# jdidion/atropos

Measured on AMD Instinct MI355X. Metric: reads/s (whole node) 150 bp SE adapter-align, higher is better.
Workload: dtype int32

## Files before the change

### atropos_amd/csrc/filter_core.hpp

```cpp
#ifndef ATR_FILTER_CORE_HPP
#define ATR_FILTER_CORE_HPP

#include "locate_core.hpp"

namespace atr {

constexpr int FILTER_MAX_M = 64;
constexpr int FILTER_CERT_T = 3;
constexpr int FILTER_CERT_TW = 6;
constexpr int FILTER_BINS = 256;

struct FilterParams {
    uint64_t peq[16];
    int rows;
    int and_mode;
    uint32_t tail;
    int32_t thr_row[FILTER_MAX_M + 1];
    uint32_t cert[FILTER_CERT_T + 1];
    uint64_t cert_sub;
    uint64_t rowsel[4];
    uint32_t tailx[3];
    uint64_t cert64[FILTER_CERT_TW + 1];
};

// ... 12 lines not shown
    const int R = m < rows ? m : rows;
    static thread_local uint8_t tab[FILTER_MAX_M + 1][FILTER_MAX_M + 1];
    uint32_t bad[FILTER_CERT_T + 1];
    for (int t = 0; t <= FILTER_CERT_T; ++t) bad[t] = 0u;
    for (int a = 1; a <= R; ++a) {
        const int xs = R - a;
        for (int y = 0; y <= R; ++y) tab[0][y] = 0;
        for (int x = 1; x <= xs; ++x) {
            tab[x][0] = 0;
            for (int y = 1; y <= R; ++y) {
                const uint8_t up = tab[x - 1][y], left = tab[x][y - 1];
                uint8_t v = up > left ? up : left;
                if (codes[a + x - 1] == codes[y - 1] && (uint8_t)(tab[x - 1][y - 1] + 1) > v) v = (uint8_t)(tab[x - 1][y - 1] + 1);
                tab[x][y] = v;
            }
        }
        for (int t = 1; t <= FILTER_CERT_T; ++t)
            for (int i = 1; i + t <= R && i < 32; ++i) {
                const int top = i + t, kk = thr_row[top];
                if (kk < t || a > top) continue;
                const int free_bases = t + kk;
                const int bound = (a < free_bases ? a : free_bases) + (int)tab[top - a][i];
                if (bound > i) bad[t] |= 1u << i;
            }
    }
    for (int t = 1; t <= FILTER_CERT_T; ++t)
        for (int i = 1; i + t <= R && i < 32; ++i)
            if (thr_row[i] >= 0 && thr_row[i + t] >= t && !((bad[t] >> i) & 1u)) cert[t] |= 1u << i;
}

inline void filter_overlap_certificates64(const uint8_t *codes, int m, int rows, const int32_t *thr_row, bool and_mode,
                                          uint64_t cert[FILTER_CERT_TW + 1]) {
    for (int t = 0; t <= FILTER_CERT_TW; ++t) cert[t] = 0ull;
    if (and_mode || rows <= 32 || rows > FILTER_MAX_M) return;
    const int R = m < rows ? m : rows;
    static thread_local uint8_t tab[FILTER_MAX_M + 1][FILTER_MAX_M + 1];
    uint64_t bad[FILTER_CERT_TW + 1];
    for (int t = 0; t <= FILTER_CERT_TW; ++t) bad[t] = 0ull;
    for (int a = 1; a <= R; ++a) {
        const int xs = R - a;
        for (int y = 0; y <= R; ++y) tab[0][y] = 0;
        for (int x = 1; x <= xs; ++x) {
            tab[x][0] = 0;
            for (int y = 1; y <= R; ++y) {
                const uint8_t up = tab[x - 1][y], left = tab[x][y - 1];
                uint8_t v = up > left ? up : left;
                if (codes[a + x - 1] == codes[y - 1] && (uint8_t)(tab[x - 1][y - 1] + 1) > v) v = (uint8_t)(tab[x - 1][y - 1] + 1);
                tab[x][y] = v;
            }
        }
        for (int t = 1; t <= FILTER_CERT_TW; ++t)
            for (int i = 1; i + t <= R && i < 64; ++i) {
                const int top = i + t, kk = thr_row[top];
                if (kk < t || a > top) continue;
                const int free_bases = t + kk;
                const int bound = (a < free_bases ? a : free_bases) + (int)tab[top - a][i];
                if (bound > i) bad[t] |= 1ull << i;
            }
    }
    for (int t = 1; t <= FILTER_CERT_TW; ++t)
        for (int i = 1; i + t <= R && i < 64; ++i)
            if (thr_row[i] >= 0 && thr_row[i + t] >= t && !((bad[t] >> i) & 1ull)) cert[t] |= 1ull << i;
}

inline uint64_t filter_substitution_certificate(const uint8_t *codes, int m, int k, bool and_mode) {
    if (and_mode || m < 8 || m > 64 || k < 1 || k > 4) return 0ull;
    for (int i = 0; i < m; ++i) if (codes[i] != 1 && codes[i] != 2 && codes[i] != 4 && codes[i] != 8) return 0ull;
    const int OLO = -3 * k, OHI = 2 * k, NO = OHI - OLO + 1;
    uint64_t cert = 0ull;
    for (int r = 1; r <= m; ++r) {
        const auto ok = [&](int i, int o) {
            const int q = i + o;
            if (q < 1 || q > m) return true;
            return q == r ? codes[i - 1] != codes[r - 1] : codes[i - 1] == codes[q - 1];
        };
        bool threat = false;
        {
            bool cur[24][5], nxt[24][5];
            for (int o = 0; o < NO; ++o) for (int b = 0; b <= k; ++b) cur[o][b] = (b == 0) && ok(1, OLO + o);
            for (int i = 2; i <= m; ++i) {
                for (int o = 0; o < NO; ++o) for (int b = 0; b <= k; ++b) nxt[o][b] = false;
                for (int o = 0; o < NO; ++o) for (int b = 0; b <= k; ++b) if (cur[o][b])
                    for (int step = 0; b + step <= k && o + step < NO; ++step) if (ok(i, OLO + o + step)) nxt[o + step][b + step] = true;
                for (int o = 0; o < NO; ++o) for (int b = 0; b <= k; ++b) cur[o][b] = nxt[o][b];
            }
            for (int o = 0; o < NO; ++o) for (int b = 0; b <= k; ++b) threat = threat || cur[o][b];
        }
        for (int o = -2 * k; o <= -1 && !threat; ++o) {
            int bad = 0;
            for (int i = 1; i <= m; ++i) bad += ok(i, o) ? 0 : 1;
            threat = bad <= 1;
        }
        for (int o = -2 * k; o <= 0 && !threat; ++o)
            for (int x = 1; x <= m && !threat; ++x) {
                bool all = true;
                for (int i = 1; i <= m && all; ++i) if (i != x) all = ok(i, i < x ? o : o - 1);
                threat = all;
            }
        if (!threat) cert |= 1ull << (r - 1);
    }
    return cert;
}

inline FilterParams filter_params(const uint64_t *peq64, const uint8_t *codes, int m, int flags, bool and_mode,
                                  const int16_t *thr, int min_overlap, bool planes_path = false) {
    FilterParams fp;
    fp.rows = m; fp.and_mode = and_mode ? 1 : 0; fp.tail = 0u;
    fp.tailx[0] = fp.tailx[1] = fp.tailx[2] = 0u;
    for (int i = 0; i <= FILTER_MAX_M; ++i)
        fp.thr_row[i] = (i >= 1 && i <= m && i >= min_overlap && ((flags & ATR_STOP_WITHIN_SEQ1) || i == m)) ? (int32_t)thr[i] : -1;
    for (int c = 0; c < 16; ++c) fp.peq[c] = peq64[c];
    (void)planes_path;
    if (filter_narrow_applies(m, flags)) {
        fp.rows = FILTER_NARROW_ROWS;
        for (int c = 0; c < 16; ++c) fp.peq[c] = (peq64[c] >> (64 - m)) & 0xFFFFFFFFull;
        for (int t = 0; t < m - FILTER_NARROW_ROWS; ++t) {
            const uint32_t nib = (uint32_t)(codes[FILTER_NARROW_ROWS + t] & 15u) << (4 * (t & 7));
            if (t < 8) fp.tail |= nib; else fp.tailx[(t >> 3) - 1] |= nib;
        }
    }
    filter_overlap_certificates(codes, m, fp.rows, fp.thr_row, and_mode, fp.cert);
    filter_overlap_certificates64(codes, m, planes_path ? fp.rows : 0, fp.thr_row, and_mode, fp.cert64);
    fp.cert_sub = 0ull;
    fp.rowsel[0] = fp.rowsel[1] = fp.rowsel[2] = fp.rowsel[3] = 0ull;
    if (m <= FILTER_MAX_M && (flags & ATR_STOP_WITHIN_SEQ2) && !(flags & ATR_START_WITHIN_SEQ1) && m >= min_overlap && thr[m] >= 1) {
        const int k = (int)thr[m];
        fp.cert_sub = filter_substitution_certificate(codes, m, k, and_mode);
        if (fp.cert_sub)
            for (int i = 0; i < m; ++i) fp.rowsel[codes[i] == 1 ? 0 : codes[i] == 2 ? 1 : codes[i] == 4 ? 2 : 3] |= 1ull << i;
    }
    return fp;
}

constexpr int BAND_W = 16;
#ifndef ATR_BAND_INTERSECT
#define ATR_BAND_INTERSECT 1
#endif
ATR_DEV uint32_t window_word(int j_lo, int j_hi, bool scan, int rows, bool band) {
    return 0x80000000u | (uint32_t)j_lo | ((uint32_t)j_hi << 10) | (scan ? (1u << 20) : 0u) | ((uint32_t)rows << 21) |
           (band ? (1u << 28) : 0u);
}
ATR_DEV bool window_band(uint32_t w) { return ((w >> 28) & 1u) != 0; }
ATR_DEV int window_rows(uint32_t w) { return (int)((w >> 21) & 0x7Fu); }
ATR_DEV int window_lo(uint32_t w) { return (int)(w & 0x3FFu); }
ATR_DEV int window_hi(uint32_t w) { return (int)((w >> 10) & 0x3FFu); }
ATR_DEV bool window_scan(uint32_t w) { return ((w >> 20) & 1u) != 0; }
ATR_DEV bool window_valid(uint32_t w) { return (w >> 31) != 0; }
ATR_DEV uint32_t last_band_word(int dlo, int top, int span, int width, bool rowm) {
    return window_word(dlo, span | (width << 6), true, top, true) | (rowm ? (1u << 29) : 0u);
}
ATR_DEV int last_band_span(uint32_t w) { return window_hi(w) & 63; }
ATR_DEV int last_band_width(uint32_t w) { return window_hi(w) >> 6; }
ATR_DEV bool last_band_rowm(uint32_t w) { return ((w >> 29) & 1u) != 0; }
constexpr int BAND_BINS = 96, ROWS_BIN0 = 192;
ATR_DEV int triangle_rows(int rows, int n, int j, int k) { return rows - (n - j) + k; }
ATR_DEV bool ragged_rows_bins(bool start_within_seq1) { return !start_within_seq1; }
constexpr int TAIL_COLUMNS = 64;

constexpr int LAST_BIN0 = 32;
ATR_DEV int window_bin(uint32_t w, int m, bool by_rows) {
    const int rows = window_rows(w), start = window_lo(w) >> 3;
    if (window_band(w)) {
        if (window_scan(w)) return LAST_BIN0 + 63 - atr_min(rows, 63);
        const int wide = atr_min(7, atr_max(0, (window_hi(w) - window_lo(w) - m) >> 1));
        return (7 - wide) * 4 + atr_min(3, start >> 4);
    }
    if (rows >= m || !by_rows) return 96 + start;
    return ROWS_BIN0 + atr_min(rows, 63);
}

#ifndef ATR_HOST_EMU
__device__ __forceinline__ void fetch_peq8(const uint2 *peq, uint32_t w, uint2 (&e)[8]) {
#pragma unroll
    for (int b = 0; b < 8; ++b) {
        uint32_t off;
        if (b == 0) off = (w << 3) & 0x78u;
        else asm("v_lshrrev_b32 %0, %1, %2\n\tv_and_b32 %0, 0x78, %0" : "=v"(off) : "n"(4 * b - 3), "v"(w));
        e[b] = *(const uint2 *)((const char *)peq + off);
    }
}
#endif

struct FilterState {
    uint32_t pvl, pvh, mvl, mvh;
    int score;
    uint32_t hits;
    uint32_t nz;
    int zfirst;
    int j_first, j_last;
};

ATR_DEV int filter_row_offset(int m, bool wide) { return (wide ? 64 : 32) - m; }
ATR_DEV int filter_row_offset(int m) { return filter_row_offset(m, m > 32); }

ATR_DEV void filter_init(FilterState &F, const Uniform &u, int mf, bool wide) {
    const int off = filter_row_offset(mf, wide);
    const uint32_t low = off >= 32 ? 0u : ~0u << (off & 31);
    if (wide) { F.pvl = u.sr ? 0u : low; F.pvh = u.sr ? 0u : (off > 32 ? ~0u << (off & 31) : ~0u); }
    else { F.pvl = u.sr ? 0u : low; F.pvh = 0u; }
    F.mvl = F.mvh = 0u;
    F.score = (u.sr ? 0 : mf) - (u.k + 1);
    F.hits = F.nz = 0u;
    F.zfirst = 0;
    F.j_first = F.j_last = 0;
}
ATR_DEV void filter_init(FilterState &F, const Uniform &u, int mf) { filter_init(F, u, mf, mf > 32); }

template <bool WIDE>
ATR_DEV void filter_shift_out2(uint32_t &phl, uint32_t &phh, uint32_t &mhl, uint32_t &mhh, int &score, uint32_t &hits,
                               uint32_t &nz, uint32_t kreg) {
#ifdef ATR_HOST_EMU
    hits = (hits << 1) | ((uint32_t)score >> 31);
    nz = (nz << 1) | (uint32_t)(((uint64_t)(uint32_t)score + (uint64_t)kreg) >> 32);
    const uint32_t pout = WIDE ? phh >> 31 : phl >> 31, mout = WIDE ? mhh >> 31 : mhl >> 31;
    if (WIDE) { phh = (phh << 1) | (phl >> 31); mhh = (mhh << 1) | (mhl >> 31); }
    phl <<= 1; mhl <<= 1;
    score += (int)pout - (int)mout;
#else
    uint64_t c0, c2, c3;
    uint32_t t1, t2;
    if (WIDE)
        asm("v_add_co_u32 %10, %8, %4, %4\n\t"
            "v_add_co_u32 %11, %9, %4, %12\n\t"
            "v_add_co_u32 %0, %7, %0, %0\n\t"
            "v_add_co_u32 %2, vcc, %2, %2\n\t"
            "v_addc_co_u32 %5, %8, %5, %5, %8\n\t"
            "v_addc_co_u32 %6, %9, %6, %6, %9\n\t"
            "v_addc_co_u32 %1, %7, %1, %1, %7\n\t"
            "v_addc_co_u32 %3, vcc, %3, %3, vcc\n\t"
            "s_nop 1\n\t"
            "v_addc_co_u32 %4, %7, 0, %4, %7\n\t"
            "v_subbrev_co_u32 %4, vcc, 0, %4, vcc"
            : "+v"(phl), "+v"(phh), "+v"(mhl), "+v"(mhh), "+v"(score), "+v"(hits), "+v"(nz), "=&s"(c0), "=&s"(c2), "=&s"(c3),
              "=&v"(t1), "=&v"(t2)
            : "v"(kreg) : "vcc");
    else
        asm("v_add_co_u32 %8, %6, %2, %2\n\t"
            "v_add_co_u32 %9, %7, %2, %10\n\t"
            "v_add_co_u32 %0, %5, %0, %0\n\t"
            "v_add_co_u32 %1, vcc, %1, %1\n\t"
            "v_addc_co_u32 %3, %6, %3, %3, %6\n\t"
            "v_addc_co_u32 %4, %7, %4, %4, %7\n\t"
            "v_addc_co_u32 %2, %5, 0, %2, %5\n\t"
            "v_subbrev_co_u32 %2, vcc, 0, %2, vcc"
            : "+v"(phl), "+v"(mhl), "+v"(score), "+v"(hits), "+v"(nz), "=&s"(c0), "=&s"(c2), "=&s"(c3), "=&v"(t1), "=&v"(t2)
            : "v"(kreg) : "vcc");
#endif
}

template <bool WIDE>
ATR_DEV void filter_step(FilterState &F, uint32_t eql, uint32_t eqh, uint32_t kreg) {
    const uint32_t xvl = eql | F.mvl;
    const uint32_t tl = eql & F.pvl;
    const uint32_t sl = tl + F.pvl;
    const uint32_t xhl = ((sl ^ F.pvl) | eql);
    uint32_t phl = F.mvl | ~(xhl | F.pvl);
    uint32_t mhl = F.pvl & xhl;
    uint32_t xvh = 0, phh = 0, mhh = 0;
    if (WIDE) {
        xvh = eqh | F.mvh;
        const uint32_t th = eqh & F.pvh;
        const uint32_t sh = th + F.pvh + (sl < tl ? 1u : 0u);
        const uint32_t xhh = ((sh ^ F.pvh) | eqh);
        phh = F.mvh | ~(xhh | F.pvh);
        mhh = F.pvh & xhh;
    }
    filter_shift_out2<WIDE>(phl, phh, mhl, mhh, F.score, F.hits, F.nz, kreg);
    F.pvl = mhl | ~(xvl | phl);
    F.mvl = phl & xvl;
    if (WIDE) {
        F.pvh = mhh | ~(xvh | phh);
        F.mvh = phh & xvh;
    }
}

ATR_DEV void filter_fold(FilterState &F, int j, int mf, uint32_t kreg) {
    F.hits = (F.hits << 1) | ((uint32_t)F.score >> 31);
    F.nz = (F.nz << 1) | ((uint32_t)F.score + kreg < kreg ? 1u : 0u);
    if (j < 32) { const uint32_t keep = j <= 0 ? 0u : (1u << j) - 1u; F.hits &= keep; F.nz &= keep; }
    if (F.hits != 0u) {
        const int hi = 31 - atr_clz(F.hits), lo = atr_ctz(F.hits);
        if (F.j_first == 0) F.j_first = j - hi;
        F.j_last = j - lo;
        if (F.zfirst == 0) {
            const int span = j - mf;
            const uint32_t ok = span >= 31 ? ~0u : span < 0 ? 0u : (2u << span) - 1u;
            const uint32_t z = F.hits & ~F.nz & ok;
            if (z != 0u) F.zfirst = j - (31 - atr_clz(z));
        }
    }
    F.hits = F.nz = 0u;
}

template <class T>
ATR_DEV uint32_t filter_push_le2(uint32_t q, int d1, T t1, int d2, T t2) {
#ifdef ATR_HOST_EMU
    return (q << 2) | ((uint32_t)d1 < (uint32_t)t1 ? 2u : 0u) | ((uint32_t)d2 < (uint32_t)t2 ? 1u : 0u);
#else
    uint32_t x1, x2;
    uint64_t c;
    asm("v_subrev_co_u32 %1, vcc, %5, %4\n\t"
        "v_subrev_co_u32 %2, %3, %7, %6\n\t"
        "s_nop 0\n\t"
        "v_addc_co_u32 %0, vcc, %0, %0, vcc\n\t"
        "s_nop 0\n\t"
        "v_addc_co_u32 %0, %3, %0, %0, %3"
        : "+v"(q), "=&v"(x1), "=&v"(x2), "=&s"(c) : "v"(d1), "v"((uint32_t)t1), "v"(d2), "v"((uint32_t)t2) : "vcc");
    return q;
#endif
}

template <bool WIDE, class P>
ATR_DEV int filter_last_column(const FilterState &F, const Uniform &u, const P &fp, int &cost_of_largest,
                               bool &exact, int tail_rule, int &d_mf, int &row_exact) {
    const int mf = fp.rows;
    int d = 0, largest = 0;
    exact = true;
    const int off = filter_row_offset(mf, WIDE);
    const int low_rows = WIDE ? atr_max(0, atr_min(mf, 32 - off)) : mf;
    const auto scan = [&](uint32_t pv, uint32_t mv, int first, int rows) -> uint32_t {
        uint32_t q = 0u;
        int i = 0;
#if !defined(ATR_SPEC) && !defined(ATR_HOST_EMU)
#pragma clang loop unroll(disable)
#endif
        for (; i + 2 <= rows; i += 2) {
            const int d1 = d + (int)(pv & 1u) - (int)(mv & 1u);
            const int d2 = d1 + (int)((pv >> 1) & 1u) - (int)((mv >> 1) & 1u);
            pv >>= 2; mv >>= 2;
            d = d2;
            q = filter_push_le2(q, d1, fp.thr_row[first + i] + 1, d2, fp.thr_row[first + i + 1] + 1);
        }
        if (i < rows) {
            d += (int)(pv & 1u) - (int)(mv & 1u);
            q = (q << 1) | ((uint32_t)d < (uint32_t)(fp.thr_row[first + i] + 1) ? 1u : 0u);
        }
        return q;
    };
    {
        const uint32_t q = scan(off >= 32 ? 0u : F.pvl >> (off & 31), off >= 32 ? 0u : F.mvl >> (off & 31), 1, low_rows);
        if (q != 0u) largest = low_rows - atr_ctz(q);
    }
    if (WIDE) {
        const int hoff = off > 32 ? off - 32 : 0, hrows = mf - low_rows;
        const uint32_t q = scan(F.pvh >> hoff, F.mvh >> hoff, low_rows + 1, hrows);
        if (q != 0u) largest = low_rows + hrows - atr_ctz(q);
    }
    if (WIDE) {
        const uint64_t rows = (largest >= 64 ? ~0ull : ((1ull << largest) - 1ull)) << off;
        const uint64_t pv = ((uint64_t)F.pvh << 32) | F.pvl, mv = ((uint64_t)F.mvh << 32) | F.mvl;
        cost_of_largest = atr_popc64(pv & rows) - atr_popc64(mv & rows);
    } else {
        const uint32_t rows = (largest >= 32 ? ~0u : ((1u << largest) - 1u)) << off;
        cost_of_largest = atr_popc64((uint64_t)(F.pvl & rows)) - atr_popc64((uint64_t)(F.mvl & rows));
    }
    d_mf = d;
    row_exact = largest;
    if (tail_rule != 1)
        for (int i = mf + 1; i <= u.m; ++i)
            if ((tail_rule == 2 ? d + (i - mf) : d - (i - mf)) <= fp.thr_row[i]) { largest = i; exact = false; }
    return largest;
}

ATR_DEV uint32_t read_dword(const uint32_t *q, int nchunks, int z8);
template <class P, class DW>
ATR_DEV bool filter_tail_cmp(const P &fp, int T, int jp, DW dw) {
    const uint32_t sh = 4u * (uint32_t)(jp & 7);
    bool ok = true;
    uint32_t lo = dw(jp >> 3);
#pragma unroll
    for (int q = 0; q < FILTER_NARROW_TAIL_EXT / 8; ++q) {
        if (8 * q >= T) break;
        const uint32_t hi = dw((jp >> 3) + q + 1);
        const uint32_t w = sh ? ((lo >> sh) | (hi << (32u - sh))) : lo;
        lo = hi;
        const uint32_t tw = q == 0 ? fp.tail : fp.tailx[q >= 1 ? q - 1 : 0];
        const uint32_t x = fp.and_mode ? (w & tw) : (w ^ tw);
        const int left = T - 8 * q;
        const uint32_t ones = left >= 8 ? 0x11111111u : (0x11111111u & ((1u << (4 * left)) - 1u));
        const uint32_t nz = (x | (x >> 1) | (x >> 2) | (x >> 3)) & ones;
        ok = ok && (fp.and_mode ? nz == ones : nz == 0u);
    }
    return ok;
}
template <class P>
ATR_DEV bool filter_tail_matches(const P &fp, int T, const uint32_t *q, int nchunks, int jp) {
    return filter_tail_cmp(fp, T, jp, [&](int z) { return read_dword(q, nchunks, z); });
}

ATR_DEV uint64_t filter_cert64(const FilterParams &fp, int t) { return fp.cert64[t]; }
template <class P> ATR_DEV uint64_t filter_cert64(const P &, int) { return 0ull; }

struct FilterNoDiag { ATR_DEV_MEMBER uint64_t operator()(int) const { return ~0ull; } };

template <bool WIDE, class P, class TM, class DG = FilterNoDiag>
ATR_DEV uint32_t filter_decide_tm(const FilterState &F, const Uniform &u, const P &fp, TM tm, int n, uint32_t rec[4],
                                  int s = 0, bool have_last = true, DG dg = DG(), int pa_dlo = 0, int pa_dhi = -1) {
    const int mf = fp.rows, T = u.m - mf;
    rec[0] = 0xFFFF0000u; rec[1] = 0; rec[2] = 0; rec[3] = 0;
    if (F.zfirst != 0 && u.m >= u.min_overlap) {
        const int j = F.zfirst + T;
        if (T == 0 || (j <= n && tm(j - T))) {
            rec[0] = (uint32_t)u.m << 16;
            rec[1] = (uint32_t)(j - u.m) | ((uint32_t)j << 16);
            rec[2] = (uint32_t)u.m;
            return 0;
        }
    }
    int cost_l = 0, d_mf = 0, row_e = 0;
    bool exact_l = true;
    const int tail_rule = T == 0 ? 0 : (F.j_first == 0 || F.j_last < n - T - u.k) ? 1 : F.j_first == n ? 2 : 0;
    const int row_l = have_last ? filter_last_column<WIDE>(F, u, fp, cost_l, exact_l, tail_rule, d_mf, row_e) : 0;
    const bool lastcol = row_l != 0;
    const bool rowm = F.j_first != 0 && u.m >= u.min_overlap && !(tail_rule == 2 && d_mf + T > u.k);
    if (!lastcol && !rowm) return 0;
    if (!rowm && !u.sr && exact_l && cost_l == 0) {
        rec[0] = (uint32_t)row_l << 16;
        rec[1] = (uint32_t)(n - row_l) | ((uint32_t)n << 16);
        rec[2] = (uint32_t)row_l;
        return 0;
    }
    if (!WIDE && !rowm && !u.sr && exact_l && u.indel == 1 && cost_l >= 1 && cost_l <= FILTER_CERT_T && row_l > cost_l) {
        const int i = row_l - cost_l, off = filter_row_offset(mf, false);
        const uint32_t seg = ((1u << cost_l) - 1u) << (off + i);
        if ((F.pvl & seg) == seg && ((fp.cert[cost_l] >> i) & 1u) != 0u && n - i >= s) {
            rec[0] = (uint32_t)i << 16;
            rec[1] = (uint32_t)(n - i) | ((uint32_t)n << 16);
            rec[2] = (uint32_t)i;
            return 0;
        }
    }
    if (WIDE && !rowm && !u.sr && exact_l && u.indel == 1 && cost_l >= 1 && cost_l <= FILTER_CERT_TW && row_l > cost_l) {
        const int i = row_l - cost_l, off = filter_row_offset(mf, true);
        const uint64_t seg = ((1ull << cost_l) - 1ull) << (off + i), pv = ((uint64_t)F.pvh << 32) | F.pvl;
        if ((pv & seg) == seg && ((filter_cert64(fp, cost_l) >> i) & 1ull) != 0ull && n - i >= s) {
            rec[0] = (uint32_t)i << 16;
            rec[1] = (uint32_t)(n - i) | ((uint32_t)n << 16);
            rec[2] = (uint32_t)i;
            return 0;
        }
    }
    if (!rowm && !u.sr && exact_l && u.indel == 1) {
        const int kk = atr_min(u.k, (int)fp.thr_row[row_l]), dlo = n - row_l - kk;
        if (dlo >= s && cost_l + 2 * kk <= BAND_W - 1) return last_band_word(dlo, row_l, atr_min(cost_l, row_l - 1), cost_l + 2 * kk, false);
    }
    if (rowm && lastcol && !u.sr && u.indel == 1 && row_e != 0) {
        const int top = exact_l ? row_l : u.m, r0 = atr_max(1, row_e - cost_l);
        const int dlo = atr_min(F.j_first - mf - u.k, n - top - u.k), dhi = atr_max(F.j_last - mf + u.k, n - r0 + u.k);
        if (dlo >= s && dhi - dlo <= BAND_W - 1) return last_band_word(dlo, top, top - r0, dhi - dlo, true);
    }
    int j_lo = 0x7fffffff;
    if (rowm) j_lo = F.j_first - mf - u.k;
    if (lastcol) j_lo = atr_min(j_lo, n - row_l - ((u.indel == 1 && exact_l) ? cost_l : u.k));
    j_lo = atr_max(s, j_lo);
    bool band = rowm && !lastcol && (F.j_first - mf - u.k >= s) &&
                (F.j_last - F.j_first + 2 * u.k <= BAND_W - 1);
    int band_hi = F.j_last + T;
    const bool pa = rowm && !lastcol && !u.sr && pa_dhi >= pa_dlo && pa_dlo > s;
    if (!band && pa && pa_dhi - pa_dlo <= BAND_W - 1) {
        band = true;
        j_lo = pa_dlo;
        band_hi = pa_dhi + u.m - u.k;
    } else if (band && !u.sr && u.indel == 1 && fp.cert_sub != 0ull && ((F.j_first + F.j_last) & 1) == 0 &&
        F.j_last - F.j_first <= 2 * u.k) {
        const int xc = (F.j_first + F.j_last) >> 1, d = xc - mf, j = d + u.m;
        if (d >= s && j <= n) {
            const uint64_t mm = dg(d);
            if (mm != 0ull && (mm & (mm - 1ull)) == 0ull && (mm & fp.cert_sub) != 0ull) {
                rec[0] = (uint32_t)u.m << 16;
                rec[1] = (uint32_t)d | ((uint32_t)j << 16);
                rec[2] = (uint32_t)(u.m - 1) | (1u << 16);
                return 0;
            }
        }
    }
    if (ATR_BAND_INTERSECT && band && pa) {
        const int lo = atr_max(pa_dlo, F.j_first - mf - u.k), hi = atr_min(pa_dhi + u.m - u.k, F.j_last + T);
        if (hi - (u.m - u.k) >= lo) { j_lo = lo; band_hi = hi; }
    }
    const int j_hi = lastcol ? n : band ? band_hi : atr_min(n, F.j_last + (T ? T + u.k : 0));
    return window_word(j_lo, j_hi, lastcol, rowm ? u.m : row_l, band);
}

template <bool WIDE, class P>
ATR_DEV uint32_t filter_decide(const FilterState &F, const Uniform &u, const P &fp, const uint32_t *q,
                               int nchunks, int n, uint32_t rec[4], int s = 0) {
    const int T = u.m - fp.rows;
    return filter_decide_tm<WIDE>(F, u, fp, [&](int jp) { return filter_tail_matches(fp, T, q, nchunks, jp); }, n, rec, s);
}

struct BandParams {
    uint32_t rrep[FILTER_MAX_M];
    int and_mode, noindel;
};

constexpr int BAND_STREAM = (FILTER_MAX_M + BAND_W + 7) / 8 + 1;

ATR_DEV uint32_t read_dword(const uint32_t *q, int nchunks, int z8) {
    if (z8 < 0 || z8 >= nchunks * 4) return 0u;
    return q[(size_t)(z8 >> 2) * 256 + (z8 & 3)];
}

ATR_DEV int band_stream_dwords(int m) { return atr_min(BAND_STREAM, 3 + (m >> 3)); }
ATR_DEV void band_stage(const uint32_t *q, int nchunks, int dlo, uint32_t *ns, int nss, int ndw = BAND_STREAM) {
    const int z0 = dlo >> 3;
    const uint32_t sh = 4u * (uint32_t)(dlo & 7);
    uint32_t raw[BAND_STREAM + 1];
#pragma unroll
    for (int k = 0; k <= BAND_STREAM; ++k) raw[k] = k <= ndw ? read_dword(q, nchunks, z0 + k) : 0u;
#pragma unroll
    for (int k = 0; k < BAND_STREAM; ++k)
        if (k < ndw) ns[(size_t)k * nss] = sh ? ((raw[k] >> sh) | (raw[k + 1] << (32u - sh))) : raw[k];
}

ATR_DEV uint32_t nibble_any(uint32_t v) {
    const uint32_t t = v | (v << 1);
    return t | (t << 2);
}

template <bool AND_MODE, int ND, bool PREFIX = false, class RR>
ATR_DEV void band_rows(const Uniform &u, RR rrep_of, const uint32_t *ns, int nss, uint32_t (&band)[BAND_W]) {
    const uint32_t inf = ((uint32_t)INIT_COST_CAP << CSH) | ORG_BIAS;
    uint32_t qw0 = ns[0], qw1 = ns[(size_t)nss];
    uint32_t feed = ns[(size_t)2 * nss];
    for (int i = 1; i <= u.m; ++i) {
        const uint32_t rrep = rrep_of(i);
        uint32_t m0 = nibble_any(AND_MODE ? (qw0 & rrep) : (qw0 ^ rrep));
        uint32_t m1 = ND > 8 ? nibble_any(AND_MODE ? (qw1 & rrep) : (qw1 ^ rrep)) : 0u;
        if (AND_MODE) { m0 = ~m0; m1 = ~m1; }
        uint32_t left = inf;
        if (PREFIX && i <= u.k) {
            const uint32_t col0 = ORG_BIAS | ((uint32_t)atr_min(i * u.indel, INIT_COST_CAP) << CSH);
#pragma unroll
            for (int c = 0; c < ND; ++c) {
                const int j = i + c - u.k;
                const uint32_t bit = atr_bfe1(c < 8 ? m0 : m1, 4 * (c & 7) + 3);
                const uint32_t cd = atr_mad24(bit, COST1 + MATCH1, band[c]);
                const uint32_t up = c + 1 < ND ? band[c + 1 < ND ? c + 1 : 0] : inf;
                uint32_t nw = atr_minu(atr_minu(cd, left + u.delw), up + u.insw) & ~PRIO_MASK;
                if (j <= 0) nw = j == 0 ? col0 : inf;
                band[c] = nw;
                left = nw;
            }
        } else {
#pragma unroll
            for (int c = 0; c < ND; ++c) {
                const uint32_t bit = atr_bfe1(c < 8 ? m0 : m1, 4 * (c & 7) + 3);
                const uint32_t cd = atr_mad24(bit, COST1 + MATCH1, band[c]);
                const uint32_t up = c + 1 < ND ? band[c + 1 < ND ? c + 1 : 0] : inf;
                const uint32_t nw = atr_minu(atr_minu(cd, left + u.delw), up + u.insw) & ~PRIO_MASK;
                band[c] = nw;
                left = nw;
            }
        }
        qw0 = (qw0 >> 4) | (qw1 << 28);
        qw1 = (qw1 >> 4) | (feed << 28);
        feed >>= 4;
        if ((i & 7) == 0) {
            const int k = 2 + (i >> 3);
            feed = k < BAND_STREAM ? ns[(size_t)k * nss] : 0u;
        }
    }
}

template <bool AND_MODE>
ATR_DEV void band_locate(const Uniform &u, const uint32_t *rreps, bool noindel, const uint32_t *ns, int nss, int n,
                         uint32_t ww, int smax, const int16_t *thr, uint32_t rec[4]) {
    const int dlo = window_lo(ww);
    uint32_t band[BAND_W];
#pragma unroll
    for (int c = 0; c < BAND_W; ++c) band[c] = ORG_BIAS + (uint32_t)(dlo + c);
    const auto rr = [rreps](int i) { return rreps[i - 1]; };
    if (smax < 8) band_rows<AND_MODE, 8>(u, rr, ns, nss, band);
    else if (smax < 10) band_rows<AND_MODE, 10>(u, rr, ns, nss, band);
    else if (smax < 12) band_rows<AND_MODE, 12>(u, rr, ns, nss, band);
    else if (smax < 14) band_rows<AND_MODE, 14>(u, rr, ns, nss, band);
    else band_rows<AND_MODE, 16>(u, rr, ns, nss, band);
    Best best;
    best.key = COST_FIELD_MAX - (u.m + n);
    best.word = (uint32_t)(u.m + n) << CSH;
    best.ref_stop = u.m; best.query_stop = n; best.matches = 0;
    const int cindel = noindel ? 0 : u.indel;
#pragma unroll
    for (int c = 0; c < BAND_W; ++c) {
        const int j = dlo + u.m + c;
        if (c <= smax && band[c] < u.klimit && j <= n) consider<true>(best, band[c], u.m, j, u.min_overlap, thr, cindel);
    }
    const int cost = (int)(best.word >> CSH);
    int refstart = 0, querystart = 0, refstop = -1, querystop = 0, matches = 0, errors = 0;
    if (cost != u.m + n) {
        const int origin = (int)(best.word & ORG_MASK) - (int)ORG_BIAS;
        if (origin >= 0) querystart = origin; else refstart = -origin;
        refstop = best.ref_stop; querystop = best.query_stop;
        matches = best.matches; errors = cost;
    }
    rec[0] = (uint32_t)(refstart & 0xFFFF) | ((uint32_t)(refstop & 0xFFFF) << 16);
    rec[1] = (uint32_t)(querystart & 0xFFFF) | ((uint32_t)(querystop & 0xFFFF) << 16);
    rec[2] = (uint32_t)(matches & 0xFFFF) | ((uint32_t)(errors & 0xFFFF) << 16);
    rec[3] = 0;
}


template <bool AND_MODE, int ND>
ATR_DEV void band_rows_last(const Uniform &u, const uint32_t *rreps, const uint32_t *ns, int nss, uint32_t (&band)[BAND_W],
                            int rows_max, int cap_lo, bool active, int top, int r0, int at0, int n, const int16_t *thr,
                            int cindel, Best &best) {
    const uint32_t inf = ((uint32_t)INIT_COST_CAP << CSH) | ORG_BIAS;
    uint32_t qw0 = ns[0], qw1 = ns[(size_t)nss];
    uint32_t feed = ns[(size_t)2 * nss];
    for (int i = 1; i <= rows_max; ++i) {
        const uint32_t rrep = rreps[i - 1];
        uint32_t m0 = nibble_any(AND_MODE ? (qw0 & rrep) : (qw0 ^ rrep));
        uint32_t m1 = ND > 8 ? nibble_any(AND_MODE ? (qw1 & rrep) : (qw1 ^ rrep)) : 0u;
        if (AND_MODE) { m0 = ~m0; m1 = ~m1; }
        uint32_t left = inf;
#pragma unroll
        for (int c = 0; c < ND; ++c) {
            const uint32_t bit = atr_bfe1(c < 8 ? m0 : m1, 4 * (c & 7) + 3);
            const uint32_t cd = atr_mad24(bit, COST1 + MATCH1, band[c]);
            const uint32_t up = c + 1 < ND ? band[c + 1 < ND ? c + 1 : 0] : inf;
            const uint32_t nw = atr_minu(atr_minu(cd, left + u.delw), up + u.insw) & ~PRIO_MASK;
            band[c] = nw;
            left = nw;
        }
        if (i >= cap_lo) {
            const int at = at0 - i;
            if (active && i <= top && i >= r0 && (u.er || i == u.m)) {
                uint32_t cell = band[0];
#pragma unroll
                for (int c = 1; c < ND; ++c) cell = at == c ? band[c] : cell;
                if (cell < u.klimit) consider<true>(best, cell, i, n, u.min_overlap, thr, cindel);
            }
        }
        qw0 = (qw0 >> 4) | (qw1 << 28);
        qw1 = (qw1 >> 4) | (feed << 28);
        feed >>= 4;
        if ((i & 7) == 0) {
            const int k = 2 + (i >> 3);
            feed = k < BAND_STREAM ? ns[(size_t)k * nss] : 0u;
        }
    }
}

template <bool AND_MODE>
ATR_DEV void band_locate_last(const Uniform &u, const uint32_t *rreps, bool noindel, const uint32_t *ns, int nss, int n,
                              uint32_t ww, bool active, int smax, int rows_max, int cap_lo, const int16_t *thr,
                              uint32_t rec[4]) {
    const int dlo = window_lo(ww), top = window_rows(ww), r0 = top - last_band_span(ww), at0 = n - dlo;
    uint32_t band[BAND_W];
#pragma unroll
    for (int c = 0; c < BAND_W; ++c) band[c] = ORG_BIAS + (uint32_t)(dlo + c);
    Best best, bm;
    best.key = COST_FIELD_MAX - (u.m + n);
    best.word = (uint32_t)(u.m + n) << CSH;
    best.ref_stop = u.m; best.query_stop = n; best.matches = 0;
    bm = best;
    const int cindel = noindel ? 0 : u.indel;
    if (smax < 4) band_rows_last<AND_MODE, 4>(u, rreps, ns, nss, band, rows_max, cap_lo, active, top, r0, at0, n, thr, cindel, best);
    else if (smax < 6) band_rows_last<AND_MODE, 6>(u, rreps, ns, nss, band, rows_max, cap_lo, active, top, r0, at0, n, thr, cindel, best);
    else if (smax < 8) band_rows_last<AND_MODE, 8>(u, rreps, ns, nss, band, rows_max, cap_lo, active, top, r0, at0, n, thr, cindel, best);
    else if (smax < 10) band_rows_last<AND_MODE, 10>(u, rreps, ns, nss, band, rows_max, cap_lo, active, top, r0, at0, n, thr, cindel, best);
    else if (smax < 12) band_rows_last<AND_MODE, 12>(u, rreps, ns, nss, band, rows_max, cap_lo, active, top, r0, at0, n, thr, cindel, best);
    else if (smax < 14) band_rows_last<AND_MODE, 14>(u, rreps, ns, nss, band, rows_max, cap_lo, active, top, r0, at0, n, thr, cindel, best);
    else band_rows_last<AND_MODE, 16>(u, rreps, ns, nss, band, rows_max, cap_lo, active, top, r0, at0, n, thr, cindel, best);
    if (last_band_rowm(ww) && rows_max == u.m) {
        const int width = last_band_width(ww);
#pragma unroll
        for (int c = 0; c < BAND_W; ++c) {
            const int j = dlo + u.m + c;
            if (c <= width && band[c] < u.klimit && j <= n) consider<true>(bm, band[c], u.m, j, u.min_overlap, thr, cindel);
        }
        if (bm.key >= best.key) best = bm;
    }
    const int cost = (int)(best.word >> CSH);
    int refstart = 0, querystart = 0, refstop = -1, querystop = 0, matches = 0, errors = 0;
    if (cost != u.m + n) {
        const int origin = (int)(best.word & ORG_MASK) - (int)ORG_BIAS;
        if (origin >= 0) querystart = origin; else refstart = -origin;
        refstop = best.ref_stop; querystop = best.query_stop;
        matches = best.matches; errors = cost;
    }
    rec[0] = (uint32_t)(refstart & 0xFFFF) | ((uint32_t)(refstop & 0xFFFF) << 16);
    rec[1] = (uint32_t)(querystart & 0xFFFF) | ((uint32_t)(querystop & 0xFFFF) << 16);
    rec[2] = (uint32_t)(matches & 0xFFFF) | ((uint32_t)(errors & 0xFFFF) << 16);
    rec[3] = 0;
}


inline bool prefix_band_applies(int flags, int m, int k) {
    return flags == ATR_STOP_WITHIN_SEQ2 && m <= FILTER_MAX_M && k >= 0 && k < m && 2 * k + 1 <= BAND_W;
}

template <bool AND_MODE, class RR>
ATR_DEV void band_locate_prefix_rr(const Uniform &u, RR rr, bool noindel, const uint32_t *ns, int nss, int n,
                                   const int16_t *thr, uint32_t rec[4]) {
    const int k = u.k, smax = 2 * k;
    const uint32_t inf = ((uint32_t)INIT_COST_CAP << CSH) | ORG_BIAS;
    const int max_n = atr_min(n, u.m + k);
    uint32_t band[BAND_W];
#pragma unroll
    for (int c = 0; c < BAND_W; ++c) {
        const int j = c - k;
        band[c] = j < 0 ? inf : (ORG_BIAS | ((uint32_t)atr_min(j * u.indel, INIT_COST_CAP) << CSH));
    }
    if (smax < 4) band_rows<AND_MODE, 4, true>(u, rr, ns, nss, band);
    else if (smax < 6) band_rows<AND_MODE, 6, true>(u, rr, ns, nss, band);
    else if (smax < 8) band_rows<AND_MODE, 8, true>(u, rr, ns, nss, band);
    else if (smax < 12) band_rows<AND_MODE, 12, true>(u, rr, ns, nss, band);
    else band_rows<AND_MODE, 16, true>(u, rr, ns, nss, band);
    Best best;
    best.key = COST_FIELD_MAX - (u.m + n);
    best.word = (uint32_t)(u.m + n) << CSH;
    best.ref_stop = u.m; best.query_stop = n; best.matches = 0;
    const int cindel = noindel ? 0 : u.indel;
    uint32_t last = inf;
    bool have_last = false;
#pragma unroll
    for (int c = 0; c < BAND_W; ++c) {
        const int j = u.m + c - k;
        if (c <= smax && j >= 0 && j <= max_n) {
            if (band[c] < u.klimit) consider<true>(best, band[c], u.m, j, u.min_overlap, thr, cindel);
            if (j == n) { last = band[c]; have_last = true; }
        }
    }
    if (max_n == n && have_last) consider<true>(best, last, u.m, n, u.min_overlap, thr, cindel);
    const int cost = (int)(best.word >> CSH);
    int refstart = 0, querystart = 0, refstop = -1, querystop = 0, matches = 0, errors = 0;
    if (cost != u.m + n) {
        const int origin = (int)(best.word & ORG_MASK) - (int)ORG_BIAS;
        if (origin >= 0) querystart = origin; else refstart = -origin;
        refstop = best.ref_stop; querystop = best.query_stop;
        matches = best.matches; errors = cost;
    }
    rec[0] = (uint32_t)(refstart & 0xFFFF) | ((uint32_t)(refstop & 0xFFFF) << 16);
    rec[1] = (uint32_t)(querystart & 0xFFFF) | ((uint32_t)(querystop & 0xFFFF) << 16);
    rec[2] = (uint32_t)(matches & 0xFFFF) | ((uint32_t)(errors & 0xFFFF) << 16);
    rec[3] = 0;
}

template <bool AND_MODE>
// ... 8 lines not shown
```

### atropos_amd/csrc/tail_filter.hpp

```cpp
#ifndef ATR_TAIL_FILTER_HPP
#define ATR_TAIL_FILTER_HPP

#ifdef ATR_HOST_EMU
#include "filter_core.hpp"
#else
#include "fast_work.hpp"
#endif

namespace atr {

#ifndef ATR_TAIL_ROWS_UNROLL
#define ATR_TAIL_ROWS_UNROLL 8
#endif
#ifndef ATR_TAIL_WINDOW_UNROLL
#define ATR_TAIL_WINDOW_UNROLL 2
#endif
constexpr int TAIL_ROWS_UNROLL = ATR_TAIL_ROWS_UNROLL;
static_assert(TAIL_ROWS_UNROLL >= 8 && TAIL_ROWS_UNROLL % 8 == 0, "the feed position is a compile-time place of the body");

template <bool AND_MODE, int ND>
ATR_DEV void tail_band_row(const Uniform &u, uint32_t rrep, uint32_t qw0, uint32_t qw1, uint32_t (&band)[BAND_W]) {
    const uint32_t inf = ((uint32_t)INIT_COST_CAP << CSH) | ORG_BIAS;
    uint32_t m0 = nibble_any(AND_MODE ? (qw0 & rrep) : (qw0 ^ rrep));
    uint32_t m1 = ND > 8 ? nibble_any(AND_MODE ? (qw1 & rrep) : (qw1 ^ rrep)) : 0u;
    if (AND_MODE) { m0 = ~m0; m1 = ~m1; }
    uint32_t left = inf;
#pragma unroll
    for (int c = 0; c < ND; ++c) {
        const uint32_t bit = atr_bfe1(c < 8 ? m0 : m1, 4 * (c & 7) + 3);
        const uint32_t cd = atr_mad24(bit, COST1 + MATCH1, band[c]);
        const uint32_t up = c + 1 < ND ? band[c + 1 < ND ? c + 1 : 0] : inf;
        const uint32_t nw = atr_minu(atr_minu(cd, left + u.delw), up + u.insw) & ~PRIO_MASK;
        band[c] = nw;
        left = nw;
    }
}

struct TailLast {
    int cap_lo, top, r0, at0, n, cindel;
    bool active;
};

template <bool AND_MODE, int ND, int ROWS_MAX, bool LAST>
ATR_DEV void tail_band_sweep(const Uniform &u, const uint32_t *rreps, int rows, const uint32_t *ns, int nss,
                             uint32_t (&band)[BAND_W], const TailLast &tl, const int16_t *thr, Best &best) {
    uint32_t qw0 = ns[0], qw1 = ns[(size_t)nss];
    uint32_t feed = ns[(size_t)2 * nss];
#pragma unroll 1
    for (int i0 = 0; i0 < ROWS_MAX; i0 += TAIL_ROWS_UNROLL) {
        if (i0 >= rows) break;
#pragma unroll
        for (int t = 0; t < TAIL_ROWS_UNROLL; ++t) {
            const int i = i0 + t + 1;
            if (i <= ROWS_MAX && i <= rows) {
                tail_band_row<AND_MODE, ND>(u, rreps[i - 1], qw0, qw1, band);
                if (LAST && i >= tl.cap_lo) {
                    const int at = tl.at0 - i;
                    if (tl.active && i <= tl.top && i >= tl.r0 && (u.er || i == u.m)) {
                        uint32_t cell = band[0];
#pragma unroll
                        for (int c = 1; c < ND; ++c) cell = at == c ? band[c] : cell;
                        if (cell < u.klimit) consider<true>(best, cell, i, tl.n, u.min_overlap, thr, tl.cindel);
                    }
                }
                qw0 = (qw0 >> 4) | (qw1 << 28);
                qw1 = (qw1 >> 4) | (feed << 28);
                feed >>= 4;
                if (((t + 1) & 7) == 0) {
                    const int k = 2 + (i >> 3);
                    feed = k < BAND_STREAM ? ns[(size_t)k * nss] : 0u;
                }
            }
        }
    }
}

ATR_DEV void tail_band_record(const Best &best, int none_cost, uint32_t rec[4]) {
    const int cost = (int)(best.word >> CSH);
    int refstart = 0, querystart = 0, refstop = -1, querystop = 0, matches = 0, errors = 0;
    if (cost != none_cost) {
        const int origin = (int)(best.word & ORG_MASK) - (int)ORG_BIAS;
        if (origin >= 0) querystart = origin; else refstart = -origin;
        refstop = best.ref_stop; querystop = best.query_stop;
        matches = best.matches; errors = cost;
    }
    rec[0] = (uint32_t)(refstart & 0xFFFF) | ((uint32_t)(refstop & 0xFFFF) << 16);
    rec[1] = (uint32_t)(querystart & 0xFFFF) | ((uint32_t)(querystop & 0xFFFF) << 16);
    rec[2] = (uint32_t)(matches & 0xFFFF) | ((uint32_t)(errors & 0xFFFF) << 16);
    rec[3] = 0;
}

template <bool AND_MODE, int ROWS_MAX>
ATR_DEV void tail_band_locate(const Uniform &u, const uint32_t *rreps, bool noindel, const uint32_t *ns, int nss, int n,
                              uint32_t ww, int smax, const int16_t *thr, uint32_t rec[4]) {
    const int dlo = window_lo(ww);
    uint32_t band[BAND_W];
#pragma unroll
    for (int c = 0; c < BAND_W; ++c) band[c] = ORG_BIAS + (uint32_t)(dlo + c);
    Best best;
    best.key = COST_FIELD_MAX - (u.m + n);
    best.word = (uint32_t)(u.m + n) << CSH;
    best.ref_stop = u.m; best.query_stop = n; best.matches = 0;
    const TailLast none = {0, 0, 0, 0, 0, 0, false};
    if (smax < 8) tail_band_sweep<AND_MODE, 8, ROWS_MAX, false>(u, rreps, u.m, ns, nss, band, none, thr, best);
    else if (smax < 10) tail_band_sweep<AND_MODE, 10, ROWS_MAX, false>(u, rreps, u.m, ns, nss, band, none, thr, best);
    else if (smax < 12) tail_band_sweep<AND_MODE, 12, ROWS_MAX, false>(u, rreps, u.m, ns, nss, band, none, thr, best);
    else if (smax < 14) tail_band_sweep<AND_MODE, 14, ROWS_MAX, false>(u, rreps, u.m, ns, nss, band, none, thr, best);
    else tail_band_sweep<AND_MODE, 16, ROWS_MAX, false>(u, rreps, u.m, ns, nss, band, none, thr, best);
    const int cindel = noindel ? 0 : u.indel;
#pragma unroll
    for (int c = 0; c < BAND_W; ++c) {
        const int j = dlo + u.m + c;
        if (c <= smax && band[c] < u.klimit && j <= n) consider<true>(best, band[c], u.m, j, u.min_overlap, thr, cindel);
    }
    tail_band_record(best, u.m + n, rec);
}

template <bool AND_MODE, int ROWS_MAX>
ATR_DEV void tail_band_locate_last(const Uniform &u, const uint32_t *rreps, bool noindel, const uint32_t *ns, int nss, int n,
                                   uint32_t ww, bool active, int smax, int rows_max, int cap_lo, const int16_t *thr,
                                   uint32_t rec[4]) {
    const int dlo = window_lo(ww), top = window_rows(ww), r0 = top - last_band_span(ww), at0 = n - dlo;
    uint32_t band[BAND_W];
#pragma unroll
    for (int c = 0; c < BAND_W; ++c) band[c] = ORG_BIAS + (uint32_t)(dlo + c);
    Best best, bm;
    best.key = COST_FIELD_MAX - (u.m + n);
    best.word = (uint32_t)(u.m + n) << CSH;
    best.ref_stop = u.m; best.query_stop = n; best.matches = 0;
    bm = best;
    const int cindel = noindel ? 0 : u.indel;
    const TailLast tl = {cap_lo, top, r0, at0, n, cindel, active};
    if (smax < 4) tail_band_sweep<AND_MODE, 4, ROWS_MAX, true>(u, rreps, rows_max, ns, nss, band, tl, thr, best);
    else if (smax < 6) tail_band_sweep<AND_MODE, 6, ROWS_MAX, true>(u, rreps, rows_max, ns, nss, band, tl, thr, best);
    else if (smax < 8) tail_band_sweep<AND_MODE, 8, ROWS_MAX, true>(u, rreps, rows_max, ns, nss, band, tl, thr, best);
    else if (smax < 10) tail_band_sweep<AND_MODE, 10, ROWS_MAX, true>(u, rreps, rows_max, ns, nss, band, tl, thr, best);
    else if (smax < 12) tail_band_sweep<AND_MODE, 12, ROWS_MAX, true>(u, rreps, rows_max, ns, nss, band, tl, thr, best);
    else if (smax < 14) tail_band_sweep<AND_MODE, 14, ROWS_MAX, true>(u, rreps, rows_max, ns, nss, band, tl, thr, best);
    else tail_band_sweep<AND_MODE, 16, ROWS_MAX, true>(u, rreps, rows_max, ns, nss, band, tl, thr, best);
    if (last_band_rowm(ww) && rows_max == u.m) {
        const int width = last_band_width(ww);
#pragma unroll
        for (int c = 0; c < BAND_W; ++c) {
            const int j = dlo + u.m + c;
            if (c <= width && band[c] < u.klimit && j <= n) consider<true>(bm, band[c], u.m, j, u.min_overlap, thr, cindel);
        }
        if (bm.key >= best.key) best = bm;
    }
    tail_band_record(best, u.m + n, rec);
}

#if defined(ATR_TAIL_SPEC) && !defined(ATR_HOST_EMU)
#include "tail_spec_config.h"

__device__ __forceinline__ Uniform tail_uniform() {
    Uniform u;
    u.m = tspec::M; u.k = tspec::K; u.p0 = tspec::MT - tspec::M; u.indel = tspec::INDEL; u.min_overlap = tspec::MIN_OVERLAP;
    u.sr = (tspec::FLAGS & ATR_START_WITHIN_SEQ1) != 0; u.sq = (tspec::FLAGS & ATR_START_WITHIN_SEQ2) != 0;
    u.er = (tspec::FLAGS & ATR_STOP_WITHIN_SEQ1) != 0;  u.eq = (tspec::FLAGS & ATR_STOP_WITHIN_SEQ2) != 0;
    u.first_p = u.p0 + (u.er ? 0 : u.m);
    u.insw = (uint32_t)u.indel * COST1 + PRIO_INS;
    u.delw = (uint32_t)u.indel * COST1 + PRIO_DEL;
    u.klimit = (uint32_t)(u.k + 1) << CSH;
    return u;
}

__device__ __forceinline__ int tail_lanes_per_wave(long long tasks, long long grid_waves, int fixed) {
    if (fixed) return fixed;
    int lpw = 1;
    while (lpw < 64 && (long long)lpw * grid_waves < tasks) lpw <<= 1;
    return lpw;
}

struct TailShared {
    int16_t thr[tspec::M + 2];
    uint32_t init[tspec::MT + 1];
    __attribute__((aligned(16))) uint32_t nm[16][4];
    uint32_t stream[4][BAND_STREAM][64];
    uint32_t spread[4][256];
};

__device__ __forceinline__ void tail_band_blocks(TailShared &S, int block, int nblocks, const uint4 *__restrict__ packed,
                                                 const int32_t *__restrict__ lens, int nchunks, int max_len,
                                                 uint4 *__restrict__ out, const FastWork &wk) {
    constexpr int M = tspec::M;
    const Uniform u = tail_uniform();
    const long long total = (long long)wk.binbase[BAND_BINS];
    const int lane = threadIdx.x & 63, wave = __builtin_amdgcn_readfirstlane((int)(threadIdx.x >> 6));
    const long long stride = (long long)nblocks * 4;
    const int lpw = tail_lanes_per_wave(total, stride, wk.lpw);
    const long long nwaves = (total + lpw - 1) / lpw;
    uint32_t *ns = &S.stream[wave][0][lane];
    long long wv = (long long)block * 4 + wave;
    if (wv >= nwaves) return;
    auto slot_of = [&](long long w) { return w * lpw + lane; };
    auto live_of = [&](long long w) { return w < nwaves && lane < lpw && slot_of(w) < total; };
    auto dense_of = [&](long long w, uint2 task) { return live_of(w) && (task.y & PIECE_NODENSE) == 0u; };
    const uint4 zero4 = make_uint4(0u, 0u, 0u, 0u);
    uint2 task = live_of(wv) ? wk.order[slot_of(wv)] : make_uint2(0u, 0u);
    uint32_t di = live_of(wv) ? wk.dref[slot_of(wv)] : 0u;
    uint2 task1 = live_of(wv + stride) ? wk.order[slot_of(wv + stride)] : make_uint2(0u, 0u);
    uint32_t di1 = live_of(wv + stride) ? wk.dref[slot_of(wv + stride)] : 0u;
    uint4 a = dense_of(wv, task) ? wk.tdata[2 * (size_t)di] : zero4, b = dense_of(wv, task) ? wk.tdata[2 * (size_t)di + 1] : zero4;
    int n = live_of(wv) ? (lens ? lens[task.x] : max_len) : 0;
    for (; wv < nwaves; wv += stride) {
        const bool live = live_of(wv);
        const long long r = (long long)task.x;
        const uint32_t ww = task.y;
        const bool dense1 = dense_of(wv + stride, task1);
        const uint4 a1 = dense1 ? wk.tdata[2 * (size_t)di1] : zero4, b1 = dense1 ? wk.tdata[2 * (size_t)di1 + 1] : zero4;
        const int n1 = live_of(wv + stride) ? (lens ? lens[task1.x] : max_len) : 0;
        const bool live2 = live_of(wv + 2 * stride);
        const uint2 task2 = live2 ? wk.order[slot_of(wv + 2 * stride)] : make_uint2(0u, 0u);
        const uint32_t di2 = live2 ? wk.dref[slot_of(wv + 2 * stride)] : 0u;

        const bool last = live && window_scan(ww);
        const bool any_last = wave_max_i32(last ? 1 : 0) != 0, any_rowm = wave_max_i32(live && !last ? 1 : 0) != 0;
        const int s_lane = (live && !last) ? window_hi(ww) - u.m + u.k - window_lo(ww) : 0;
        const int smax = min(BAND_W - 1, wave_max_i32(s_lane));
        const bool dense = live && (ww & PIECE_NODENSE) == 0u;
        if (dense) {
            ns[0] = a.x; ns[64] = a.y; ns[128] = a.z; ns[192] = a.w;
            ns[256] = b.x; ns[320] = b.y; ns[384] = b.z; ns[448] = b.w;
        }
        if (wave_max_i32(live && !dense ? 1 : 0) != 0) {
            const uint32_t *q = (const uint32_t *)(packed + ((size_t)(r >> 6) * nchunks) * 64 + (r & 63));
            if (live && !dense) band_stage_planes(q, nchunks, window_lo(ww), ns, 64, S.spread, band_stream_dwords(M));
        }
        uint32_t rec[4] = {0xFFFF0000u, 0u, 0u, 0u};
        if (any_rowm) tail_band_locate<tspec::AND_MODE, M>(u, tspec::RREP, tspec::NOINDEL, ns, 64, n, ww, smax, S.thr, rec);
        if (any_last) {
            const int smax_l = min(BAND_W - 1, wave_max_i32(last ? last_band_width(ww) : 0));
            const int rows_max = wave_max_i32(last ? (last_band_rowm(ww) ? u.m : window_rows(ww)) : 0);
            const int cap_lo = wave_min_i32(last ? window_rows(ww) - last_band_span(ww) : 0x7fffffff);
            uint32_t rec_l[4];
            tail_band_locate_last<tspec::AND_MODE, M>(u, tspec::RREP, tspec::NOINDEL, ns, 64, n, ww, last, smax_l, min(rows_max, M), cap_lo, S.thr, rec_l);
            if (last) { rec[0] = rec_l[0]; rec[1] = rec_l[1]; rec[2] = rec_l[2]; rec[3] = rec_l[3]; }
        }
        if (live) out[r] = make_uint4(rec[0], rec[1], rec[2], rec[3]);
        task = task1; di = di1; a = a1; b = b1; n = n1;
        task1 = task2; di1 = di2;
    }
}

template <int W>
__device__ __forceinline__ void tail_load_mask(uint32_t (&nm)[W], const uint32_t (*s_nm)[4], uint32_t q) {
#pragma unroll
    for (int w = 0; w < W; ++w) nm[w] = s_nm[q][w];
}

__device__ __forceinline__ void tail_window_blocks(TailShared &S, int block, int nblocks, const uint4 *__restrict__ packed,
                                                   const int32_t *__restrict__ lens, int nchunks, int max_len,
                                                   uint4 *__restrict__ out, const FastWork &wk) {
    constexpr int MT = tspec::MT;
    constexpr bool NOINDEL = tspec::NOINDEL;
    const Uniform u = tail_uniform();
    const int16_t *s_thr = S.thr;
    const uint32_t *s_init = S.init;
    const uint32_t (*s_nm)[4] = S.nm;
    const uint32_t (*s_spread)[256] = S.spread;
    const long long first = (long long)wk.binbase[BAND_BINS], total = (long long)wk.binbase[FILTER_BINS];
    if (total <= first) return;
    const int lane = threadIdx.x & 63;
    const int lpw = tail_lanes_per_wave(total - first, (long long)nblocks * 4, wk.lpw);
    const long long nwaves = (total - first + lpw - 1) / lpw;
    __builtin_amdgcn_s_setprio(3);
    for (long long wv = (long long)block * 4 + __builtin_amdgcn_readfirstlane((int)(threadIdx.x >> 6)); wv < nwaves;
// ... 124 lines not shown
```

Measured before the change: 25.10 billion.

## Route last-column filter cases to narrow band windows with certified fallback row

Adds two band-window paths for reads whose filter shows a row match that extends to the last column. One covers the case with no row error, estimating the first qualifying row from the per-row thresholds. The other certifies an exact or low-cost last-column candidate and encodes it as a fallback row in a band window word. The band kernels then merge that certified row into the best result instead of sending these reads to a full last-column scan. This aims to move more reads from wide scan windows to cheap banded alignment, at the cost of extra decision logic and a risk of result mismatches in edge cases.

Measured after the change: 24.97 billion. No clear change (-0.5%).

```diff
diff --git a/atropos_amd/csrc/filter_core.hpp b/atropos_amd/csrc/filter_core.hpp
--- a/atropos_amd/csrc/filter_core.hpp
+++ b/atropos_amd/csrc/filter_core.hpp
@@ -188,6 +188,22 @@
 ATR_DEV int last_band_span(uint32_t w) { return window_hi(w) & 63; }
 ATR_DEV int last_band_width(uint32_t w) { return window_hi(w) >> 6; }
 ATR_DEV bool last_band_rowm(uint32_t w) { return ((w >> 29) & 1u) != 0; }
+#ifndef ATR_BAND_FALLBACK
+#define ATR_BAND_FALLBACK 1
+#endif
+ATR_DEV uint32_t fallback_band_word(int j_lo, int band_hi, int row) {
+    return window_word(j_lo, band_hi, false, row, true) | (1u << 29);
+}
+ATR_DEV int band_fallback_row(uint32_t w) {
+    return (ATR_BAND_FALLBACK && window_band(w) && !window_scan(w) && ((w >> 29) & 1u) != 0) ? window_rows(w) : 0;
+}
+ATR_DEV void band_fallback_merge(Best &best, int row, int n) {
+    const int key = (row << 12) | COST_FIELD_MAX;
+    if (row != 0 && key > best.key) {
+        best.key = key; best.word = ORG_BIAS + (uint32_t)(n - row);
+        best.ref_stop = row; best.query_stop = n; best.matches = row;
+    }
+}
 constexpr int BAND_BINS = 96, ROWS_BIN0 = 192;
 ATR_DEV int triangle_rows(int rows, int n, int j, int k) { return rows - (n - j) + k; }
 ATR_DEV bool ragged_rows_bins(bool start_within_seq1) { return !start_within_seq1; }
@@ -426,6 +442,8 @@
 
 ATR_DEV uint64_t filter_cert64(const FilterParams &fp, int t) { return fp.cert64[t]; }
 template <class P> ATR_DEV uint64_t filter_cert64(const P &, int) { return 0ull; }
+ATR_DEV bool filter_band_fallback(const FilterParams &) { return ATR_BAND_FALLBACK != 0; }
+template <class P> ATR_DEV bool filter_band_fallback(const P &) { return false; }
 
 struct FilterNoDiag { ATR_DEV_MEMBER uint64_t operator()(int) const { return ~0ull; } };
 
@@ -485,19 +503,46 @@
         const int dlo = atr_min(F.j_first - mf - u.k, n - top - u.k), dhi = atr_max(F.j_last - mf + u.k, n - r0 + u.k);
         if (dlo >= s && dhi - dlo <= BAND_W - 1) return last_band_word(dlo, top, top - r0, dhi - dlo, true);
     }
+    if (filter_band_fallback(fp) && rowm && lastcol && !u.sr && u.indel == 1 && row_e == 0) {
+        int r0 = u.m;
+        for (int i = u.m - 1; i > mf; --i)
+            if ((tail_rule == 2 ? d_mf + (i - mf) : d_mf - (i - mf)) <= fp.thr_row[i]) r0 = i;
+        const int dlo = atr_min(F.j_first - mf - u.k, n - u.m - u.k), dhi = atr_max(F.j_last - mf + u.k, n - r0 + u.k);
+        if (dlo >= s && dhi - dlo <= BAND_W - 1) return last_band_word(dlo, u.m, u.m - r0, dhi - dlo, true);
+    }
+    int fb = 0;
+    if (filter_band_fallback(fp) && rowm && lastcol && !u.sr && u.indel == 1 && exact_l) {
+        if (cost_l == 0) fb = row_l;
+        else if (row_l > cost_l && cost_l <= (WIDE ? FILTER_CERT_TW : FILTER_CERT_T)) {
+            const int i = row_l - cost_l, off = filter_row_offset(mf, WIDE);
+            bool ok;
+            if (WIDE) {
+                const uint64_t seg = ((1ull << cost_l) - 1ull) << (off + i), pv = ((uint64_t)F.pvh << 32) | F.pvl;
+                ok = (pv & seg) == seg && ((filter_cert64(fp, cost_l) >> i) & 1ull) != 0ull;
+            } else {
+                const uint32_t seg = ((1u << cost_l) - 1u) << (off + i);
+                ok = (F.pvl & seg) == seg && ((fp.cert[cost_l] >> i) & 1u) != 0u;
+            }
+            if (ok) fb = i;
+        }
+        const bool fits = (F.j_first - mf - u.k >= s) && (F.j_last - F.j_first + 2 * u.k <= BAND_W - 1);
+        const bool pfits = pa_dhi >= pa_dlo && pa_dlo > s && pa_dhi - pa_dlo <= BAND_W - 1;
+        if (n - fb < s || !(fits || pfits)) fb = 0;
+    }
+    const bool rowm_only = rowm && (!lastcol || fb != 0);
     int j_lo = 0x7fffffff;
     if (rowm) j_lo = F.j_first - mf - u.k;
-    if (lastcol) j_lo = atr_min(j_lo, n - row_l - ((u.indel == 1 && exact_l) ? cost_l : u.k));
+    if (lastcol && fb == 0) j_lo = atr_min(j_lo, n - row_l - ((u.indel == 1 && exact_l) ? cost_l : u.k));
     j_lo = atr_max(s, j_lo);
-    bool band = rowm && !lastcol && (F.j_first - mf - u.k >= s) &&
+    bool band = rowm_only && (F.j_first - mf - u.k >= s) &&
                 (F.j_last - F.j_first + 2 * u.k <= BAND_W - 1);
     int band_hi = F.j_last + T;
-    const bool pa = rowm && !lastcol && !u.sr && pa_dhi >= pa_dlo && pa_dlo > s;
+    const bool pa = rowm_only && !u.sr && pa_dhi >= pa_dlo && pa_dlo > s;
     if (!band && pa && pa_dhi - pa_dlo <= BAND_W - 1) {
         band = true;
         j_lo = pa_dlo;
         band_hi = pa_dhi + u.m - u.k;
-    } else if (band && !u.sr && u.indel == 1 && fp.cert_sub != 0ull && ((F.j_first + F.j_last) & 1) == 0 &&
+    } else if (band && fb == 0 && !u.sr && u.indel == 1 && fp.cert_sub != 0ull && ((F.j_first + F.j_last) & 1) == 0 &&
         F.j_last - F.j_first <= 2 * u.k) {
         const int xc = (F.j_first + F.j_last) >> 1, d = xc - mf, j = d + u.m;
         if (d >= s && j <= n) {
@@ -514,6 +559,7 @@
         const int lo = atr_max(pa_dlo, F.j_first - mf - u.k), hi = atr_min(pa_dhi + u.m - u.k, F.j_last + T);
         if (hi - (u.m - u.k) >= lo) { j_lo = lo; band_hi = hi; }
     }
+    if (fb != 0) return fallback_band_word(j_lo, band_hi, fb);
     const int j_hi = lastcol ? n : band ? band_hi : atr_min(n, F.j_last + (T ? T + u.k : 0));
     return window_word(j_lo, j_hi, lastcol, rowm ? u.m : row_l, band);
 }
@@ -622,6 +668,7 @@
         const int j = dlo + u.m + c;
         if (c <= smax && band[c] < u.klimit && j <= n) consider<true>(best, band[c], u.m, j, u.min_overlap, thr, cindel);
     }
+    band_fallback_merge(best, band_fallback_row(ww), n);
     const int cost = (int)(best.word >> CSH);
     int refstart = 0, querystart = 0, refstop = -1, querystop = 0, matches = 0, errors = 0;
     if (cost != u.m + n) {
diff --git a/atropos_amd/csrc/tail_filter.hpp b/atropos_amd/csrc/tail_filter.hpp
--- a/atropos_amd/csrc/tail_filter.hpp
+++ b/atropos_amd/csrc/tail_filter.hpp
@@ -113,6 +113,7 @@
         const int j = dlo + u.m + c;
         if (c <= smax && band[c] < u.klimit && j <= n) consider<true>(best, band[c], u.m, j, u.min_overlap, thr, cindel);
     }
+    band_fallback_merge(best, band_fallback_row(ww), n);
     tail_band_record(best, u.m + n, rec);
 }
 
```
